# tyb311/TCCT

Measured on AMD Instinct MI355X. Metric: OCT B-scans/sec fwd+bwd(+clip+AdamW), stc_tt bs=8 1x800x1100, higher is better.
Workload: dtype bf16; 1 GPU; stc_tt --los=di bs=8/GPU 1x800x1100 (net tensors 3x800x1104); global_batch=8, parallelism=dp1, ranks=1, grad_allreduce=none, slowest_step=101

## Files before the change

include/tcct_hip.h:

```cpp
#ifndef TCCT_HIP_H
#define TCCT_HIP_H
#include <stdint.h>
#ifdef __cplusplus
extern "C" {
#endif

typedef void* tcct_stream_t;

enum { TCCT_F32 = 0, TCCT_BF16 = 1 };
enum { TCCT_ACT_NONE = 0, TCCT_ACT_LRELU = 1, TCCT_ACT_HSWISH = 2, TCCT_ACT_GELU = 3, TCCT_ACT_SIGMOID = 4,
       TCCT_ACT_ABS = 5 };
enum { TCCT_CRIT_DICE = 0, TCCT_CRIT_DICE2 = 1, TCCT_CRIT_IOU = 2, TCCT_CRIT_MSE = 3 };
enum { TCCT_MCRIT_DICE = 0, TCCT_MCRIT_DICE2 = 1, TCCT_MCRIT_IOU = 2, TCCT_MCRIT_CE = 3 };

int tcct_version(void);
const char* tcct_last_error(void);
int tcct_set_outputs_prezeroed(int on);

int tcct_image_to_nhwc4(const float* img, void* out, int N, int Csrc, int H, int Wsrc, int Wdst, int dtype,
                        tcct_stream_t stream);
int tcct_u8_gather2d(const uint8_t* src, uint8_t* dst, int N, int SH, int SW, int C, int sy0, int sx0, int sh, int sw, int DH, int DW,
                     int dy0, int dx0, int dh, int dw, int flipy, int flipx, int mul, int div, int fill, tcct_stream_t stream);
int tcct_onehot_to_index(const int64_t* onehot, uint8_t* lab, int N, int C, int64_t HW, tcct_stream_t stream);
int tcct_labels_to_u8(const int64_t* lab, uint8_t* out, int N, int H, int Wsrc, int Wdst, tcct_stream_t stream);
int tcct_nhwc_to_nchw_f32(const void* x, float* y, int N, int64_t HW, int C, int dtype, tcct_stream_t stream);

int tcct_act_fwd(const void* x, void* y, int64_t n, int kind, int dtype, tcct_stream_t stream);
int tcct_act_bwd(const void* x, const void* dy, void* dx, int64_t n, int kind, int dtype, tcct_stream_t stream);
int tcct_add(const void* a, const void* b, void* y, int64_t n, int dtype, tcct_stream_t stream);
int tcct_add_act_fwd(const void* a, const void* b, void* y, int64_t n, int kind, int dtype, tcct_stream_t stream);
int tcct_add_act_bwd(const void* a, const void* b, const void* dy, void* dx, int64_t n, int kind, int dtype,
                     tcct_stream_t stream);
int tcct_residual_fwd(const void* x, const void* z, const float* scale, void* y, int B, int64_t per_sample,
                      int dtype, tcct_stream_t stream);
int tcct_scale_rows(const void* x, const float* scale, void* y, int B, int64_t per_sample, int dtype,
                    tcct_stream_t stream);
int tcct_affine2_add(const void* y1, const float* ab1, const void* y2, const float* ab2, void* z, int64_t M, int C, int dtype, tcct_stream_t stream);
int tcct_add3_scale(const void* a, const void* b, const void* c, void* y, int64_t n, float alpha, int dtype,
                    tcct_stream_t stream);
int tcct_scale(const void* x, void* y, int64_t n, float alpha, int dtype, tcct_stream_t stream);
int tcct_concat2(const void* a, const void* b, void* y, int64_t M, int Ca, int Cb, int dtype, tcct_stream_t stream);
int tcct_split2(const void* dy, void* da, void* db, int64_t M, int Ca, int Cb, int dtype, tcct_stream_t stream);
int tcct_axpy_f32(const float* x, float* y, int64_t n, float alpha, tcct_stream_t stream);

int tcct_bn_stats(const void* x, int64_t M, int C, int pre_act, double* sums , int dtype, tcct_stream_t stream);
int tcct_bn_finalize(const double* sums, int64_t M, int C, const float* gamma, const float* beta, float eps,
                     float momentum, float* running_mean, float* running_var, int64_t* num_batches_tracked,
                     float* mean_rstd , float* ab , tcct_stream_t stream);
int tcct_bn_eval_ab(int C, const float* gamma, const float* beta, float eps, const float* running_mean,
                    const float* running_var, float* mean_rstd, float* ab, tcct_stream_t stream);
int tcct_bn_apply(const void* x, void* y, int64_t M, int C, const float* ab, int pre_act, int post_act, int dtype,
                  tcct_stream_t stream);
int tcct_bn_apply_train(const void* x, const void* res, void* y, int64_t M, int C, const double* sums, const float* gamma,
                        const float* beta, float eps, float momentum, float* running_mean, float* running_var,
                        int64_t* num_batches_tracked, float* mean_rstd, float* ab, int pre_act, int post_act, int dtype,
                        tcct_stream_t stream);
int tcct_bn_pool_fwd_train(const void* x, void* z, void* pooled, void* amax, int N, int H, int W, int C, const double* sums, const float* gamma,
                           const float* beta, float eps, float momentum, float* running_mean, float* running_var,
                           int64_t* num_batches_tracked, float* mean_rstd, float* ab, int pre_act, int post_act, int dtype,
                           tcct_stream_t stream);
int tcct_bn_pool_bwd(const void* x, const void* dpool, const void* dskip, const void* amax, void* dx, int N, int H, int W, int C, const float* mean_rstd,
                     const float* ab, int pre_act, int post_act, double* sums, float* dgamma, float* dbeta, int dtype, tcct_stream_t stream);
int tcct_bn_apply_add(const void* x, const void* res, void* y, int64_t M, int C, const float* ab, int pre_act, int post_act, int dtype,
                      tcct_stream_t stream);
int tcct_bn_bwd_reduce(const void* x, const void* dy, int64_t M, int C, const float* mean_rstd, const float* ab,
                       int pre_act, int post_act, double* sums , int dtype, tcct_stream_t stream);
int tcct_bn_bwd_apply(const void* x, const void* dy, void* dx, int64_t M, int C, const float* mean_rstd,
                      const float* ab, const float* gamma, const double* sums, int pre_act, int post_act,
                      float* dgamma, float* dbeta, int dtype, tcct_stream_t stream);
int tcct_bn_bwd_coef(const double* sums, int raw, int64_t M, int C, const float* mean_rstd, const float* ab, float* coef, float* dgamma,
                     float* dbeta, tcct_stream_t stream);
int tcct_bn_bwd_reduce2_raw(const void* y1, const void* y2, const void* dz, int64_t M, int C, double* raw1, double* raw2, int dtype, tcct_stream_t stream);
int tcct_bn_sums_from_raw(const double* raw, const float* mean_rstd, int C, double* sums, tcct_stream_t stream);

int tcct_bn2_add_act_fwd(const void* xa, const void* xb, void* y, int64_t M, int C, const float* abA, const float* abB, int pre_act,
                         int act, int dtype, tcct_stream_t stream);
int tcct_bn2_add_act_train(const void* xa, const void* xb, void* y, int64_t M, int C, const double* sumsA, const float* gammaA,
                           const float* betaA, float* running_meanA, float* running_varA, int64_t* nbtA, float* mean_rstdA,
                           float* abA, const double* sumsB, const float* gammaB, const float* betaB, float* running_meanB,
                           float* running_varB, int64_t* nbtB, float* mean_rstdB, float* abB, float eps, float momentum,
                           int pre_act, int act, int dtype, tcct_stream_t stream);
int tcct_bn2_add_act_bwd_reduce(const void* xa, const void* xb, const void* dy, int64_t M, int C, const float* mean_rstdA,
                                const float* abA, const float* mean_rstdB, const float* abB, int pre_act, int act, double* sums,
                                int dtype, tcct_stream_t stream);
int tcct_bn2_add_act_bwd_apply(const void* xa, const void* xb, const void* dy, void* dxa, void* dxb, int64_t M, int C,
                               const float* mean_rstdA, const float* abA, const float* mean_rstdB, const float* abB,
                               const double* sums, int pre_act, int act, float* dgammaA, float* dbetaA, float* dgammaB,
                               float* dbetaB, int dtype, tcct_stream_t stream);

int tcct_layernorm_fwd(const void* x, void* y, int64_t M, int C, const float* gamma, const float* beta, float eps,
                       float* mean_rstd , int dtype, tcct_stream_t stream);
int tcct_layernorm_bwd(const void* x, const void* dy, void* dx, int64_t M, int C, const float* gamma,
                       const float* mean_rstd, float* dgamma, float* dbeta, int dtype, tcct_stream_t stream);
int tcct_layernorm_bwd_add(const void* x, const void* dy, const void* res, void* dx, int64_t M, int C, const float* gamma,
                           const float* mean_rstd, float* dgamma, float* dbeta, int dtype, tcct_stream_t stream);

int tcct_conv2d_fwd(const void* x, const float* w, const float* bias, void* y, int N, int H, int W, int Cin,
                    int Cin_w, int Cout, int KH, int KW, int stride, int padh, int padw, int in_dtype, int out_dtype,
                    tcct_stream_t stream);
int tcct_conv2d_dgrad(const void* dy, const float* w, void* dx, int N, int H, int W, int Cin, int Cout, int KH,
                      int KW, int padh, int padw, int dy_dtype, int dx_dtype, tcct_stream_t stream);
int tcct_conv2d_wgrad(const void* x, const void* dy, float* dw, float* dbias, int N, int H, int W, int Cin,
                      int Cin_w, int Cout, int KH, int KW, int stride, int padh, int padw, int x_dtype, int dy_dtype,
                      tcct_stream_t stream);

int tcct_conv32f_pack_weights(const float* w, float* wp, int KH, int KW, int transposed, tcct_stream_t stream);
int tcct_conv32f_fwd(const float* x, const float* wp, const float* bias, const float* yadd, float* y, int N, int H, int W, int KH, int KW, int PH,
                     int PW, tcct_stream_t stream);
int tcct_conv32f_wgrad(const float* x, const float* dy, float* dw, float* dbias, int N, int H, int W, int KH, int KW, int PH, int PW,
                       tcct_stream_t stream);
int tcct_conv32f_pack_weights_sub(const float* w, float* wp, int KH, int KW, int transposed, int cin_total, int o_off, int i_off, tcct_stream_t stream);
int tcct_conv32f_fwd_strided(const float* x, const float* wp, const float* bias, float* y, int N, int H, int W, int KH, int KW, int PH, int PW, int xs,
                             int xo, int ys, int yo, int accumulate, tcct_stream_t stream);
int tcct_conv32f_wgrad_strided(const float* x, const float* dy, float* dw, float* dbias, int N, int H, int W, int KH, int KW, int PH, int PW, int xs,
                               int xo, int ds, int dof, int ldi, int o_off, int i_off, tcct_stream_t stream);
// ... 296 lines not shown
```

tcct_amd/csrc/norm.hip:

```cpp
#include "common.h"
#include <cstdlib>

#define NB 256
#define NBR 1024
static inline int bn_vec(int C, int dtype) {
    static int v8 = -1;
    if (v8 < 0) v8 = 0;
    return (v8 && dtype == TCCT_BF16 && C % 8 == 0) ? 8 : ((C % 4 == 0) ? 4 : 1);
}

template <int VEC>
__device__ __forceinline__ void bn_block_reduce2(float* sm, const float* s, const float* q, int t, int C, int CV, int R, double* sums) {
#pragma unroll
    for (int pass = 0; pass < 2; ++pass) {
        if (pass) __syncthreads();
#pragma unroll
        for (int k = 0; k < VEC; ++k) sm[t * VEC + k] = pass ? q[k] : s[k];
        __syncthreads();
        if (t < C) {
            double a = 0.0;
            const int cvv = t / VEC, k = t % VEC;
            for (int rr = 0; rr < R; ++rr) a += (double)sm[(rr * CV + cvv) * VEC + k];
            atomicAdd(&sums[pass * C + t], a);
        }
// ... 448 lines not shown
                        float dz = e[q].v[k] + (((am >> (2 * k)) & 3u) == (unsigned)q ? g.v[k] : 0.f);
                        if (POST != TCCT_ACT_NONE) dz *= actg<POST>(post_act, a_[k] * u + b_[k]);
                        s[k] += dz; q2[k] += dz * (u - mu[k]) * rs[k];
                    }
            }
        }
    }
    bn_block_reduce2<4>(sm, s, q2, t, C, C4, R, sums);
}
template <typename T, int PRE, int POST>
__global__ void k_bn_pool_bwd_apply(const T* __restrict__ x, const T* __restrict__ dpool, const T* __restrict__ dskip,
                                    const unsigned char* __restrict__ amax, T* __restrict__ dx, int N, int H, int W, int C,
                                    const float* __restrict__ mean_rstd, const float* __restrict__ ab, const double* __restrict__ sums,
                                    int pre_act, int post_act, float* __restrict__ dgamma, float* __restrict__ dbeta) {
    const int C4 = C >> 2, Ho = H >> 1, Wo = W >> 1;
    const int i = blockIdx.x * blockDim.x + threadIdx.x;
    if (blockIdx.x == 0 && blockIdx.y == 0 && threadIdx.x < C) { dbeta[threadIdx.x] = (float)sums[threadIdx.x]; dgamma[threadIdx.x] = (float)sums[C + threadIdx.x]; }
    if (i >= Wo * C4) return;
    const int wo = i / C4, c0 = (i - wo * C4) * 4;
    const float invM = 1.f / (float)((int64_t)N * H * W);
    float a_[4], b_[4], mu[4], rs[4], s1[4], s2[4];
#pragma unroll
    for (int k = 0; k < 4; ++k) {
        const int c = c0 + k;
        a_[k] = ab[c]; b_[k] = ab[C + c]; mu[k] = mean_rstd[c]; rs[k] = mean_rstd[C + c];
        s1[k] = (float)sums[c] * invM; s2[k] = (float)sums[C + c] * invM;
    }
    for (int row = blockIdx.y; row < N * Ho; row += gridDim.y) {
        const int n = row / Ho, ho = row - n * Ho;
        const int64_t b00 = (((int64_t)n * H + 2 * ho) * W + 2 * wo) * C + c0;
        const int64_t offs[4] = {b00, b00 + C, b00 + (int64_t)W * C, b00 + (int64_t)W * C + C};
        f4 v[4], e[4];
#pragma unroll
        for (int q = 0; q < 4; ++q) { v[q] = ld4(x + offs[q]); e[q] = dskip ? ld4(dskip + offs[q]) : f4zero(); }
        const int64_t p = (int64_t)row * Wo + wo;
        const f4 g = ld4(dpool + p * C + c0);
        const unsigned am = amax[p * C4 + (c0 >> 2)];
#pragma unroll
        for (int q = 0; q < 4; ++q) {
            f4 o;
#pragma unroll
            for (int k = 0; k < 4; ++k) {
                const float u = actf<PRE>(pre_act, v[q].v[k]);
                float dz = e[q].v[k] + (((am >> (2 * k)) & 3u) == (unsigned)q ? g.v[k] : 0.f);
                if (POST != TCCT_ACT_NONE) dz *= actg<POST>(post_act, a_[k] * u + b_[k]);
                const float xh = (u - mu[k]) * rs[k];
                o.v[k] = a_[k] * (dz - s1[k] - xh * s2[k]);
                if (PRE != TCCT_ACT_NONE) o.v[k] *= actg<PRE>(pre_act, v[q].v[k]);
            }
            st4(dx + offs[q], o);
        }
    }
}
static bool bn_pool_ok(int N, int H, int W, int C) { return C % 4 == 0 && C >= 4 && C <= NB && NB % (C / 4) == 0 && H % 2 == 0 && W % 2 == 0 && H >= 2 && W >= 2 && N >= 1; }
static inline dim3 bn_pool_grid(int per_row, int64_t rows) {
    const int gx = (per_row + NB - 1) / NB;
    int64_t gy = ((1 << 14) + gx - 1) / gx;
    if (gy > rows) gy = rows;
    if (gy > 65535) gy = 65535;
    if (gy < 1) gy = 1;
    return dim3((unsigned)gx, (unsigned)gy);
}
#define BN_POOL_KINDS(CALL) do { if (pre_act == TCCT_ACT_LRELU && post_act == TCCT_ACT_NONE) { constexpr int PRE = TCCT_ACT_LRELU, POST = TCCT_ACT_NONE; CALL; } \
                                 else { constexpr int PRE = -1, POST = -1; CALL; } } while (0)
extern "C" int tcct_bn_pool_fwd_train(const void* x, void* z, void* pooled, void* amax, int N, int H, int W, int C, const double* sums,
                                      const float* gamma, const float* beta, float eps, float momentum, float* running_mean,
                                      float* running_var, int64_t* num_batches_tracked, float* mean_rstd, float* ab, int pre_act, int post_act,
                                      int dtype, tcct_stream_t stream) {
    TCCT_CHECK(bn_pool_ok(N, H, W, C), "bn_pool_fwd_train: needs even H, W and C/4 dividing 256 (got %d,%d,%d)", H, W, C);
    TCCT_CHECK(sums && gamma && beta && mean_rstd && ab && amax, "bn_pool_fwd_train: NULL argument");
    BnTrain tr{sums, gamma, beta, eps, momentum, running_mean, running_var, num_batches_tracked, mean_rstd, ab};
    BN_POOL_KINDS(TCCT_DISPATCH(dtype, hipLaunchKernelGGL((k_bn_pool_fwd<T, PRE, POST>), bn_pool_grid((W / 2) * (C / 4), (int64_t)N * (H / 2)), dim3(NB), 0,
                                                          (hipStream_t)stream, (const T*)x, (T*)z, (T*)pooled, (unsigned char*)amax, N, H, W, C, pre_act, post_act, tr)));
    TCCT_LAUNCH_OK();
}
extern "C" int tcct_bn_pool_bwd(const void* x, const void* dpool, const void* dskip, const void* amax, void* dx, int N, int H, int W, int C,
                                const float* mean_rstd, const float* ab, int pre_act, int post_act, double* sums, float* dgamma, float* dbeta,
                                int dtype, tcct_stream_t stream) {
    TCCT_CHECK(bn_pool_ok(N, H, W, C), "bn_pool_bwd: needs even H, W and C/4 dividing 256 (got %d,%d,%d)", H, W, C);
    TCCT_CHECK(dpool != nullptr && amax != nullptr, "bn_pool_bwd: dpool / amax is NULL");
    hipStream_t st = (hipStream_t)stream;
    if (!tcct_skip_zero_fill() && hipMemsetAsync(sums, 0, sizeof(double) * 2 * C, st) != hipSuccess) { tcct_set_error("bn_pool_bwd: memset failed"); return -2; }
    const int64_t rows = (int64_t)N * (H / 2);
    const int gr = rows < 512 ? (int)rows : 512;
    BN_POOL_KINDS(TCCT_DISPATCH(dtype, hipLaunchKernelGGL((k_bn_pool_bwd_reduce<T, PRE, POST>), dim3(gr), dim3(NBR), 0, st, (const T*)x, (const T*)dpool,
                                                          (const T*)dskip, (const unsigned char*)amax, N, H, W, C, mean_rstd, ab, pre_act, post_act, sums)));
    BN_POOL_KINDS(TCCT_DISPATCH(dtype, hipLaunchKernelGGL((k_bn_pool_bwd_apply<T, PRE, POST>), bn_pool_grid((W / 2) * (C / 4), rows), dim3(NB), 0, st, (const T*)x,
                                                          (const T*)dpool, (const T*)dskip, (const unsigned char*)amax, (T*)dx, N, H, W, C, mean_rstd, ab, sums,
                                                          pre_act, post_act, dgamma, dbeta)));
    TCCT_LAUNCH_OK();
}

#define LN_MAXCH 3
#ifndef LN_TOK
#define LN_TOK 1
#endif
template <typename T, int NCH>
__global__ void k_ln_fwd(const T* __restrict__ x, T* __restrict__ y, int64_t M, int C, const float* __restrict__ gamma,
                         const float* __restrict__ beta, float eps, float* __restrict__ mean_rstd) {
    const int C4 = C >> 2;
    const int lane = threadIdx.x & 15;
    const int64_t grp = ((int64_t)blockIdx.x * blockDim.x + threadIdx.x) >> 4;
    const int64_t ngrp = ((int64_t)gridDim.x * blockDim.x) >> 4;
    float gam[NCH][4], bet[NCH][4];
#pragma unroll
    for (int j = 0; j < NCH; ++j)
#pragma unroll
        for (int k = 0; k < 4; ++k) {
            const int ch = lane + 16 * j;
            gam[j][k] = ch < C4 ? gamma[ch * 4 + k] : 0.f; bet[j][k] = ch < C4 ? beta[ch * 4 + k] : 0.f;
        }
    for (int64_t m0 = grp * LN_TOK; m0 < M; m0 += ngrp * LN_TOK) {
        f4 v[LN_TOK][NCH];
#pragma unroll
        for (int t = 0; t < LN_TOK; ++t)
#pragma unroll
            for (int j = 0; j < NCH; ++j) {
                const int ch = lane + 16 * j;
                if (ch < C4 && m0 + t < M) v[t][j] = ld4(x + (m0 + t) * C + ch * 4); else v[t][j] = f4zero();
            }
#pragma unroll
        for (int t = 0; t < LN_TOK; ++t) {
            const int64_t m = m0 + t;
            float s = 0.f;
#pragma unroll
            for (int j = 0; j < NCH; ++j) s += v[t][j].v[0] + v[t][j].v[1] + v[t][j].v[2] + v[t][j].v[3];
            s = row16_sum(s);
            float mean = s / (float)C, q = 0.f;
#pragma unroll
            for (int j = 0; j < NCH; ++j) {
                int ch = lane + 16 * j;
                if (ch < C4) {
#pragma unroll
                    for (int k = 0; k < 4; ++k) { float d = v[t][j].v[k] - mean; q += d * d; }
                }
            }
            q = row16_sum(q);
            float rstd = rsqrtf(q / (float)C + eps);
            if (m < M) {
                if (lane == 0) { mean_rstd[2 * m] = mean; mean_rstd[2 * m + 1] = rstd; }
#pragma unroll
                for (int j = 0; j < NCH; ++j) {
                    int ch = lane + 16 * j;
                    if (ch < C4) {
// ... 299 lines not shown
```

tcct_amd/ops.py:

```python
import os
import weakref

import torch

from ._lib import lib, dtype_code, TcctError, launch_on, F32, BF16

ACT = {None: 0, 'none': 0, 'lrelu': 1, 'hswish': 2, 'gelu': 3, 'sigmoid': 4, 'abs': 5}


class _ZeroPool:

    def __init__(self):
        self.buf = None
        self.off = 0
        self.active = False
        self.frozen = False

    def begin(self, device, nbytes=8 << 20):
        if self.buf is None or self.buf.device != device or self.buf.numel() < nbytes:
            if self.frozen:
                raise TcctError('the zero pool cannot be re-allocated after a training step was captured into a hipGraph '
                                f'(pool on {self.buf.device}, step on {device})')
            self.buf = torch.empty(nbytes, device=device, dtype=torch.uint8)
        self.buf.zero_()
# ... 107 lines not shown
        lib.bilinear_bwd_x2(int(BILINEAR_BWD_X2))
        _BILINEAR_X2_SET[0] = BILINEAR_BWD_X2
    fpl_lazy_grad_reset()
    _pack_evict()
    _pack_all(device)
    _STEP['main'] = torch.cuda.current_stream(device)
    for v in _STEP['marks'].values():
        v[0] = v[1] = 0


_STEP = {'main': None, 'marks': {}, 'listener': None}


def set_grad_mark_listener(fn):
    _STEP['listener'] = fn
    _STEP['marks'].clear()


def step_streams():
    out = [] if _STEP['main'] is None else [_STEP['main']]
    for v in _SIDE_STREAMS.values():
        out.append(v[0] if isinstance(v, tuple) else v)
    return out


class _FastFunction(torch.autograd.Function):

    @classmethod
    def apply(cls, *args):
        return super(torch.autograd.Function, cls).apply(*args)


class _GradMark(_FastFunction):
    @staticmethod
    def forward(ctx, x, key):
        ctx.key = key
        return x.view_as(x)

    @staticmethod
    def backward(ctx, dy):
        cnt = _STEP['marks'].get(ctx.key)
        fn = _STEP['listener']
        if cnt is not None and fn is not None:
            cnt[1] += 1
            if cnt[1] == cnt[0]:
                fn(ctx.key)
        return dy, None


def grad_mark(x, key):
    if _STEP['listener'] is None or not ZERO.active or not (torch.is_grad_enabled() and x.requires_grad):
        return x
    _STEP['marks'].setdefault(key, [0, 0])[0] += 1
    return _GradMark.apply(x, key)


def end_step():
    ZERO.end()
    if _WGRAD_USED:
        cur = torch.cuda.current_stream()
        for st in _WGRAD_USED.values():
            cur.wait_stream(st)
        _WGRAD_USED.clear()
    _WGRAD_KEEP.clear()


_WGRAD_USED = {}
_WGRAD_KEEP = []
DW_WGRAD_SIDE = True


def fresh_stream(device=None, avoid=()):
    taken = {torch.cuda.current_stream(device).cuda_stream}
    for v in _SIDE_STREAMS.values():
        taken.add((v[0] if isinstance(v, tuple) else v).cuda_stream)
    for st in avoid:
        taken.add(st.cuda_stream)
    for _ in range(64):
        st = torch.cuda.Stream(device=device)
        if st.cuda_stream not in taken:
            return st
    raise TcctError('fresh_stream: no stream of the pool is free of aliases')


class _wgrad_stream:
    def __init__(self, enable, *tensors):
        self.enable, self.tensors = enable, tensors

    def __enter__(self):
        if not self.enable:
            return self
        cur = torch.cuda.current_stream()
        key = ('wgrad', cur.device.index)
        ent = _SIDE_STREAMS.get(key)
        if ent is None:
            ent = _SIDE_STREAMS[key] = (fresh_stream(cur.device), torch.cuda.Event())
        self.side, ev = ent
        ev.record(cur)
        self.side.wait_event(ev)
        self.ctx = launch_on(self.side)
        self.ctx.__enter__()
        return self

    def __exit__(self, *exc):
        if not self.enable:
            return False
        self.ctx.__exit__(*exc)
# ... 1007 lines not shown

    @staticmethod
    def backward(ctx, dl, _dv):
        v, skip, wa, wb = ctx.saved_tensors
        w1, b1, w2, b2, w3, b3 = ctx.params
        N_, H, W_, C, Ho, Wo, align, nc = ctx.cfg
        dl = _as(dl, torch.float32)
        dev = v.device
        M = N_ * Ho * Wo
        dv, dskip = torch.empty_like(v), torch.empty_like(skip)
        F32_, BF_ = dtype_code(torch.float32), dtype_code(v.dtype)
        lib.conv2d_dgrad(dl, wa, dv, N_, Ho, Wo, 32, nc, 1, 1, 0, 0, F32_, BF_)
        lib.conv2d_dgrad(dl, wb, dskip, N_, Ho, Wo, 32, nc, 1, 1, 0, 0, F32_, BF_)
        dy = torch.empty((N_, H, W_, C), device=dev, dtype=v.dtype)
        lib.bilinear_bwd(dv, dy, N_, H, W_, C, Ho, Wo, align, BF_)
        params = (w1, b1, w2, b2, w3, b3)
        with _wgrad_stream(_slot_written(*params), v, skip, dl, wa, wb):
            dwa, dwb = ZERO.get((nc, 32), torch.float32, dev), ZERO.get((nc, 32), torch.float32, dev)
            dccc = ZERO.get((nc,), torch.float32, dev)
            lib.pw_wgrad_smalln(v, dl, dwa, dccc, M, 32, nc, BF_, F32_)
            lib.pw_wgrad_smalln(skip, dl, dwb, None, M, 32, nc, BF_, F32_)
            outs = [_grad_out(p, tuple(p.shape)) for p in params]
            lib.tail_compose3_bwd(w1, b1, w2, b2, w3, nc, dwa, dwb, dccc, *outs)
        return (dy, dskip) + tuple(_ret(o, p) for o, p in zip(outs, params)) + (None,)


class _UpSkipConvT32AuxLow(_FastFunction):

    @staticmethod
    def forward(ctx, y, skip, w1, b1, w2, b2, w3, b3, align):
        _chk(y, skip, w1, b1, w2, b2, w3, b3)
        N_, H, W_, C = y.shape
        _, Ho, Wo, _ = skip.shape
        dev, nc = y.device, w3.shape[0]
        F32_ = dtype_code(torch.float32)
        wcc = torch.empty((nc, 64), device=dev, dtype=torch.float32)
        wa8 = torch.zeros((8, 32, 1, 1), device=dev, dtype=torch.float32)
        wa, wb = wa8[:nc], torch.empty((nc, 32, 1, 1), device=dev, dtype=torch.float32)
        ccc = torch.empty(nc, device=dev, dtype=torch.float32)
        lib.tail_compose3(w1, b1, w2, b2, w3, b3, nc, wcc, wa, wb, ccc)
        lg = torch.empty((N_, Ho, Wo, nc), device=dev, dtype=torch.float32)
        if HEAD_UPADD and align and Ho == 2 * H and Wo == 2 * W_:
            z8 = torch.empty((N_, H, W_, 8), device=dev, dtype=torch.float32)
            lib.pw_fwd(y, wa8, None, z8, N_ * H * W_, 32, 8, 0, F32_)
            lib.pw_fwd_f32_upadd(skip, wb, ccc, lg, N_, H, W_, 32, nc, z8)
        else:
            z = torch.empty((N_, H, W_, nc), device=dev, dtype=torch.float32)
            lib.pw_fwd(y, wa, None, z, N_ * H * W_, 32, nc, 0, F32_)
            lib.pw_fwd(skip, wb, ccc, lg, N_ * Ho * Wo, 32, nc, 0, F32_)
            lib.bilinear_add_fwd(z, lg, lg, N_, H, W_, nc, Ho, Wo, int(align), F32_)
        ctx.save_for_backward(y, skip, wa, wb)
        ctx.params = (w1, b1, w2, b2, w3, b3)
        ctx.cfg = (N_, H, W_, C, Ho, Wo, int(align), nc)
        return lg

    @staticmethod
    def backward(ctx, dl):
        y, skip, wa, wb = ctx.saved_tensors
        N_, H, W_, C, Ho, Wo, align, nc = ctx.cfg
        dl = _as(dl, torch.float32)
        dev = y.device
        F32_, BF_ = dtype_code(torch.float32), dtype_code(y.dtype)
        dz = torch.empty((N_, H, W_, nc), device=dev, dtype=torch.float32)
        lib.bilinear_bwd(dl, dz, N_, H, W_, nc, Ho, Wo, align, F32_)
        dy, dskip = torch.empty_like(y), torch.empty_like(skip)
        lib.conv2d_dgrad(dz, wa, dy, N_, H, W_, 32, nc, 1, 1, 0, 0, F32_, BF_)
        lib.conv2d_dgrad(dl, wb, dskip, N_, Ho, Wo, 32, nc, 1, 1, 0, 0, F32_, BF_)
        params = ctx.params
        with _wgrad_stream(_slot_written(*params), y, skip, dl, dz, wa, wb):
            dwa, dwb = ZERO.get((nc, 32), torch.float32, dev), ZERO.get((nc, 32), torch.float32, dev)
            dccc = ZERO.get((nc,), torch.float32, dev)
            lib.pw_wgrad_smalln(y, dz, dwa, None, N_ * H * W_, 32, nc, BF_, F32_)
            lib.pw_wgrad_smalln(skip, dl, dwb, dccc, N_ * Ho * Wo, 32, nc, BF_, F32_)
            outs = [_grad_out(p, tuple(p.shape)) for p in params]
            lib.tail_compose3_bwd(params[0], params[1], params[2], params[3], params[4], nc, dwa, dwb, dccc, *outs)
        return (dy, dskip) + tuple(_ret(o, p) for o, p in zip(outs, params)) + (None,)


HEAD_UPADD = True
TAIL_AUX_LOW = True


def up_skip_conv_t32_aux_low(y, skip, w1, b1, w2, b2, w3, b3, align_corners=True):
    return _UpSkipConvT32AuxLow.apply(y, skip, w1, b1, w2, b2, w3, b3, bool(align_corners))


def up_skip_conv_t32_from_y(y, skip, w1, b1, w2, b2, align_corners=True):
    with torch.no_grad():
        N_, H, W_, C = y.shape
        v = torch.empty_like(skip)
        lib.bilinear_fwd(y, v, N_, H, W_, C, skip.shape[1], skip.shape[2], int(align_corners), dtype_code(y.dtype))
    return up_skip_conv_t32_from_v(v, skip, w1, b1, w2, b2)


TAIL_AUX = True


def up_skip_conv_t32_aux_ok(y, skip, w1, b1, w2, b2, w3, b3):
    return (TAIL_AUX and up_skip_conv_t32_ok(y, skip, w1, b1, w2, b2) and w3.dim() == 4 and tuple(w3.shape[1:]) == (32, 1, 1) and 2 <= w3.shape[0] <= 8
            and b3 is not None and w3.is_contiguous())


def up_skip_conv_t32_aux(y, skip, w1, b1, w2, b2, w3, b3, align_corners=True):
    return _UpSkipConvT32Aux.apply(y, skip, w1, b1, w2, b2, w3, b3, bool(align_corners))


def up_skip_conv_t32_from_v(v, skip, w1, b1, w2, b2):
    with torch.no_grad():
        wc = torch.empty((32, 64), device=v.device, dtype=torch.float32)
        c = torch.empty(32, device=v.device, dtype=torch.float32)
        lib.tail_compose(w1, b1, w2, b2, wc, c)
        g = torch.empty_like(skip)
        lib.pw_fwd_cat2(v, skip, 32, wc, c, g, v.numel() // 32, 64, 32, None, 0)
    return g


class _HeadThroughT32(_FastFunction):

    @staticmethod
    def forward(ctx, s, wt, bt, wa, ba):
        _chk(s, wt, bt, wa, ba)
        N_, H, W_, _ = s.shape
        dev, nc = s.device, wa.shape[0]
        wh = torch.empty((nc, 32, 1, 1), device=dev, dtype=torch.float32)
        ch = torch.empty(nc, device=dev, dtype=torch.float32)
        lib.head_compose(wt, bt, wa, ba, nc, wh, ch)
        lg = torch.empty((N_, H, W_, nc), device=dev, dtype=torch.float32)
        lib.pw_fwd(s, wh, ch, lg, N_ * H * W_, 32, nc, 0, dtype_code(torch.float32))
        ctx.save_for_backward(s, wh)
        ctx.params = (wt, bt, wa, ba)
        return lg

    @staticmethod
# ... 539 lines not shown
    return (BN_DEFER and BN_FUSE and bn_training and torch.is_grad_enabled() and x.dtype == torch.bfloat16 and x.dim() == 4 and x.shape[-1] in (64, 96)
            and ACT[post_act] == ACT['hswish'] and x.numel() * 2 < 2 ** 31)


def batchnorm_deferred(x, gamma, beta, running_mean, running_var, num_batches_tracked, eps, momentum, post_act):
    link = BnLink(None, None, ACT[post_act])
    y = _BatchNormDeferred.apply(x, gamma, beta, running_mean, running_var, num_batches_tracked, float(eps), float(momentum), ACT[post_act], link)
    return y, link


def pw_conv_bn_ok(x, w, bias, bn_training, pre_act, post_act, x2=None, prev=None):
    if not (BN_FUSE and bn_training and torch.is_grad_enabled() and ACT[pre_act] == 0):
        return False
    if x.dtype != torch.bfloat16 or x.dim() != 4 or not x.is_cuda or (w.dim() == 4 and tuple(w.shape[2:]) != (1, 1)):
        return False
    K = x.shape[-1] + (x2.shape[-1] if x2 is not None else 0)
    N = w.shape[0]
    if x2 is not None and not (x.shape[-1] == 64 and x2.shape == x.shape and x2.dtype == x.dtype):
        return False
    M = x.numel() // x.shape[-1]
    if w.shape[1] != K or M * max(K, N) * 2 >= 2 ** 31:
        return False
    return bool(lib.pw_bwd_bn_supported(K, N, ACT[post_act], -1 if prev is None else prev.post, 1 if x2 is not None else 0))


def pw_conv_bn(x, w, bias, bn, post_act=None, residual=None, fork=False, x2=None, x_final=False, deferred=None, defer_apply=False):
    gamma, beta, rm, rv, nbt, eps, mom = bn
    link = BnLink(None, None, ACT[post_act])
    w4 = w.view(w.shape[0], w.shape[1], 1, 1) if w.dim() == 2 else w
    if deferred is not None:
        if post_act is not None or fork or x2 is not None or x.shape[-1] != w.shape[0] or x.shape[-1] not in (64, 96):
            raise TcctError('pw_conv_bn(deferred=...): square 64 / 96 convolution without activation, fork or concatenation only')
        prev = deferred if (x.shape[-1] == 64 and BN_FUSE_RED) else None
        out = _PwConvBN.apply(x, None, w4, bias, gamma, beta, rm, rv, nbt, float(eps), float(mom), 0, residual, False, link, prev, deferred.ab)
        out._bn_link = link
        return out
    prev = _bn_link_of(x, x_final)
    if prev is not None and not pw_conv_bn_ok(x, w, bias, True, None, post_act, x2, prev):
        prev = None
    if defer_apply:
        if residual is not None or x2 is not None or ACT[post_act] not in (ACT['hswish'], ACT['none']):
            raise TcctError('pw_conv_bn(defer_apply=True): BatchNorm (+ Hardswish) without residual / concatenation only')
        out = _PwConvBN.apply(x, None, w4, bias, gamma, beta, rm, rv, nbt, float(eps), float(mom), ACT[post_act], None, fork, link, prev, None, True)
        return out, link
    out = _PwConvBN.apply(x, x2, w4, bias, gamma, beta, rm, rv, nbt, float(eps), float(mom), ACT[post_act], residual, fork, link, prev)
    z = out[0] if fork else out
    z._bn_link = link
    return out


BN_POOL_FUSE = True


class _BnPoolFork(_FastFunction):

    @staticmethod
    def forward(ctx, x, gamma, beta, rm, rv, nbt, eps, momentum, pre, post):
        ctx.set_materialize_grads(False)
        _chk(x, gamma, beta)
        N, H, W, C = x.shape
        dc = dtype_code(x.dtype)
        fused = getattr(x, '_bn_sums', None)
        if fused is not None and fused[1] == pre and fused[0].numel() == 2 * C:
            sums = fused[0]
        else:
            sums = ZERO.get((2 * C,), torch.float64, x.device)
            lib.bn_stats(x, N * H * W, C, pre, sums, dc)
        mean_rstd = torch.empty(2 * C, device=x.device, dtype=torch.float32)
        ab = torch.empty(2 * C, device=x.device, dtype=torch.float32)
        z = torch.empty_like(x)
        pooled = torch.empty((N, H // 2, W // 2, C), device=x.device, dtype=x.dtype)
        amax = torch.empty((N, H // 2, W // 2, C // 4), device=x.device, dtype=torch.uint8)
        lib.bn_pool_fwd_train(x, z, pooled, amax, N, H, W, C, sums, gamma, beta, eps, momentum, rm, rv, nbt, mean_rstd, ab, pre, post, dc)
        ctx.save_for_backward(x, mean_rstd, ab, amax)
        ctx.cfg = (pre, post, gamma, beta)
        return pooled, z

    @staticmethod
    def backward(ctx, dpool, dskip):
        x, mean_rstd, ab, amax = ctx.saved_tensors
        pre, post, gamma, beta = ctx.cfg
        N, H, W, C = x.shape
        dc = dtype_code(x.dtype)
        if dpool is None and dskip is None:
            return (None,) * 10
        if dpool is None:
            dpool = torch.zeros((N, H // 2, W // 2, C), device=x.device, dtype=x.dtype)
        dpool = _as(dpool, x.dtype)
        if dskip is not None:
            dskip = _as(dskip, x.dtype)
        sums = ZERO.get((2 * C,), torch.float64, x.device)
        dx = torch.empty_like(x)
        dg = _grad_out(gamma) if ZERO.active and getattr(gamma, '_grad_slot', None) is not None else torch.empty(C, device=x.device, dtype=torch.float32)
        db = _grad_out(beta) if ZERO.active and getattr(beta, '_grad_slot', None) is not None else torch.empty(C, device=x.device, dtype=torch.float32)
        lib.bn_pool_bwd(x, dpool, dskip, amax, dx, N, H, W, C, mean_rstd, ab, pre, post, sums, dg, db, dc)
        return dx, _ret(dg, gamma), _ret(db, beta), None, None, None, None, None, None, None


def bn_pool_ok(x, training):
    N, H, W, C = x.shape
    return (BN_POOL_FUSE and training and torch.is_grad_enabled() and x.requires_grad and C % 4 == 0 and C <= 256 and 256 % (C // 4) == 0
            and H % 2 == 0 and W % 2 == 0 and H >= 2 and W >= 2)


def batchnorm_maxpool2_fork(x, gamma, beta, running_mean, running_var, num_batches_tracked=None, eps=1e-5, momentum=0.1, pre_act=None,
                            post_act=None):
    return _BnPoolFork.apply(x, gamma, beta, running_mean, running_var, num_batches_tracked, float(eps), float(momentum), ACT[pre_act], ACT[post_act])


def batchnorm(x, gamma, beta, running_mean, running_var, num_batches_tracked=None, eps=1e-5, momentum=0.1,
              pre_act=None, post_act=None, training=True, residual=None):
    if not training and torch.is_grad_enabled() and x.requires_grad:
        raise TcctError('eval-mode batchnorm is inference-only here')
    link = None
    if (BN_FUSE and training and torch.is_grad_enabled() and x.dtype == torch.bfloat16 and ACT[pre_act] == 0
            and ACT[post_act] in (0, 2) and x.shape[-1] in (64, 96, 128)):
        link = BnLink(None, None, ACT[post_act])
    z = _BatchNorm.apply(x, gamma, beta, running_mean, running_var, num_batches_tracked, float(eps), float(momentum),
                         ACT[pre_act], ACT[post_act], bool(training), residual, link)
    if link is not None:
        z._bn_link = link
    return z


class _Bn2AddAct(_FastFunction):

    @staticmethod
    def forward(ctx, xa, gA, bA, xb, gB, bB, bufs, eps, momentum, pre, act_kind):
        _chk(xa, xb, gA, bA, gB, bB)
        C = xa.shape[-1]
        M = xa.numel() // C
        dc = dtype_code(xa.dtype)
        st, ss = [], []
        for x, g, b, (rm, rv, nbt) in ((xa, gA, bA, bufs[0]), (xb, gB, bB, bufs[1])):
            fused = getattr(x, '_bn_sums', None)
            if fused is not None and fused[1] == pre and fused[0].numel() == 2 * C:
                sums = fused[0]
            else:
                sums = ZERO.get((2 * C,), torch.float64, x.device)
                lib.bn_stats(x, M, C, pre, sums, dc)
            mr = torch.empty(2 * C, device=x.device, dtype=torch.float32)
            ab = torch.empty(2 * C, device=x.device, dtype=torch.float32)
            st += [mr, ab]
            ss.append(sums)
        y = torch.empty_like(xa)
        (rmA, rvA, nbtA), (rmB, rvB, nbtB) = bufs
        lib.bn2_add_act_train(xa, xb, y, M, C, ss[0], gA, bA, rmA, rvA, nbtA, st[0], st[1], ss[1], gB, bB, rmB, rvB, nbtB, st[2], st[3],
                              eps, momentum, pre, act_kind, dc)
        ctx.save_for_backward(xa, xb, *st)
        ctx.cfg = (pre, act_kind)
        ctx.params = (gA, bA, gB, bB)
        return y

    @staticmethod
    def backward(ctx, dy):
        xa, xb, mrA, abA, mrB, abB = ctx.saved_tensors
        pre, act_kind = ctx.cfg
        gA, bA, gB, bB = ctx.params
        dy = _as(dy, xa.dtype)
        C = xa.shape[-1]
# ... 1192 lines not shown
```

Baseline: 423.5 B-scans/s.

## Fuse low-rank skip dgrad into batchnorm-maxpool backward kernels

Instead of materializing the full-resolution skip gradient through a separate 1x1 conv dgrad (nc->32 channels) and reading it back in the BN+pool backward, the head's backward passes a recipe (dl, wb, nc) through a link object attached to the skip tensor. New HIP reduce and apply kernels recompute dskip on the fly from the small nc-channel gradient staged in LDS, rounding to bf16 to match the old path. This removes a full-size bf16 tensor write and read plus a kernel launch. In exchange it adds cross-autograd plumbing through a zero-stride marker tensor and recomputes the tiny matmul in both the reduce and apply passes.

Measured after the change: 429.6 B-scans/s (median of 6 runs). 1.01x the previous value.

```diff
diff --git a/include/tcct_hip.h b/include/tcct_hip.h
--- a/include/tcct_hip.h
+++ b/include/tcct_hip.h
@@ -61,6 +61,9 @@
                            tcct_stream_t stream);
 int tcct_bn_pool_bwd(const void* x, const void* dpool, const void* dskip, const void* amax, void* dx, int N, int H, int W, int C, const float* mean_rstd,
                      const float* ab, int pre_act, int post_act, double* sums, float* dgamma, float* dbeta, int dtype, tcct_stream_t stream);
+int tcct_bn_pool_bwd_lowrank(const void* x, const void* dpool, const float* dl, const float* wb, int nc, const void* amax, void* dx, int N, int H, int W,
+                             int C, const float* mean_rstd, const float* ab, int pre_act, int post_act, double* sums, float* dgamma, float* dbeta,
+                             int dtype, tcct_stream_t stream);
 int tcct_bn_apply_add(const void* x, const void* res, void* y, int64_t M, int C, const float* ab, int pre_act, int post_act, int dtype,
                       tcct_stream_t stream);
 int tcct_bn_bwd_reduce(const void* x, const void* dy, int64_t M, int C, const float* mean_rstd, const float* ab,
diff --git a/tcct_amd/csrc/norm.hip b/tcct_amd/csrc/norm.hip
--- a/tcct_amd/csrc/norm.hip
+++ b/tcct_amd/csrc/norm.hip
@@ -524,6 +524,141 @@
         }
     }
 }
+#define LR_SLOT 256
+template <int NC>
+__device__ __forceinline__ void lowrank_stage(float* __restrict__ slot, const float* __restrict__ dl0 , int64_t row_stride ,
+                                              int nwin , int lane) {
+    wave_lds_fence();
+    if (lane < nwin * NC) {
+        const float2 r0 = reinterpret_cast<const float2*>(dl0)[lane], r1 = reinterpret_cast<const float2*>(dl0 + row_stride)[lane];
+        reinterpret_cast<float2*>(slot)[lane] = r0;
+        reinterpret_cast<float2*>(slot + LR_SLOT / 2)[lane] = r1;
+    }
+    wave_lds_fence();
+}
+template <int NC>
+__device__ __forceinline__ void lowrank_dskip(const float* __restrict__ slot, int wl, const float (&w)[NC][4], f4 (&e)[4]) {
+#pragma unroll
+    for (int rr = 0; rr < 2; ++rr) {
+        float f[2 * NC];
+#pragma unroll
+        for (int i = 0; i < NC; ++i) {
+            const float2 t = reinterpret_cast<const float2*>(slot + rr * (LR_SLOT / 2) + wl * 2 * NC)[i];
+            f[2 * i] = t.x; f[2 * i + 1] = t.y;
+        }
+#pragma unroll
+        for (int col = 0; col < 2; ++col) {
+            float a[4] = {0.f, 0.f, 0.f, 0.f};
+#pragma unroll
+            for (int j = 0; j < NC; ++j)
+#pragma unroll
+                for (int k = 0; k < 4; ++k) a[k] += f[col * NC + j] * w[j][k];
+            const uint32_t lo = pack_bf16x2(a[0], a[1]), hi = pack_bf16x2(a[2], a[3]);
+            f4& o = e[rr * 2 + col];
+            o.v[0] = __uint_as_float(lo << 16); o.v[1] = __uint_as_float(lo & 0xffff0000u);
+            o.v[2] = __uint_as_float(hi << 16); o.v[3] = __uint_as_float(hi & 0xffff0000u);
+        }
+    }
+}
+template <int NC>
+__global__ void __launch_bounds__(NBR) k_bn_pool_bwd_reduce_lr(const bf16* __restrict__ x, const bf16* __restrict__ dpool, const float* __restrict__ dl,
+                                                               const float* __restrict__ wb, const unsigned char* __restrict__ amax, int N, int H, int W,
+                                                               const float* __restrict__ mean_rstd, double* __restrict__ sums) {
+    constexpr int C = 32, C4 = 8, R = NBR / C4;
+    __shared__ __attribute__((aligned(16))) float sm[NBR * 4];
+    const int Ho = H >> 1, Wo = W >> 1;
+    const int t = threadIdx.x, lane = t & 63, wl = lane >> 3, cv = t & 7, c0 = cv * 4;
+    float* slot = sm + (t >> 6) * LR_SLOT;
+    float s[4], q2[4], mu[4], rs[4], w[NC][4];
+#pragma unroll
+    for (int k = 0; k < 4; ++k) { s[k] = q2[k] = 0.f; mu[k] = mean_rstd[c0 + k]; rs[k] = mean_rstd[C + c0 + k]; }
+#pragma unroll
+    for (int j = 0; j < NC; ++j)
+#pragma unroll
+        for (int k = 0; k < 4; ++k) w[j][k] = wb[j * C + c0 + k];
+    for (int row = blockIdx.x; row < N * Ho; row += gridDim.x) {
+        const int n = row / Ho, ho = row - n * Ho;
+        for (int wo0 = (t >> 6) * 8; wo0 < Wo; wo0 += R) {
+            const int wo = wo0 + wl;
+            const int64_t pix0 = ((int64_t)n * H + 2 * ho) * W + 2 * wo0;
+            lowrank_stage<NC>(slot, dl + pix0 * NC, (int64_t)W * NC, min(8, Wo - wo0), lane);
+            if (wo >= Wo) continue;
+            const int64_t b00 = (pix0 + 2 * wl) * C + c0;
+            const int64_t offs[4] = {b00, b00 + C, b00 + (int64_t)W * C, b00 + (int64_t)W * C + C};
+            f4 v[4], e[4];
+#pragma unroll
+            for (int q = 0; q < 4; ++q) v[q] = ld4(x + offs[q]);
+            const int64_t p = (int64_t)row * Wo + wo;
+            const f4 g = ld4(dpool + p * C + c0);
+            const unsigned am = amax[p * C4 + cv];
+            lowrank_dskip<NC>(slot, wl, w, e);
+#pragma unroll
+            for (int q = 0; q < 4; ++q)
+#pragma unroll
+                for (int k = 0; k < 4; ++k) {
+                    const float u = actf<TCCT_ACT_LRELU>(TCCT_ACT_LRELU, v[q].v[k]);
+                    const float dz = e[q].v[k] + (((am >> (2 * k)) & 3u) == (unsigned)q ? g.v[k] : 0.f);
+                    s[k] += dz; q2[k] += dz * (u - mu[k]) * rs[k];
+                }
+        }
+    }
+    __syncthreads();
+    bn_block_reduce2<4>(sm, s, q2, t, C, C4, R, sums);
+}
+template <int NC>
+__global__ void __launch_bounds__(NB) k_bn_pool_bwd_apply_lr(const bf16* __restrict__ x, const bf16* __restrict__ dpool, const float* __restrict__ dl,
+                                                             const float* __restrict__ wb, const unsigned char* __restrict__ amax, bf16* __restrict__ dx,
+                                                             int N, int H, int W, const float* __restrict__ mean_rstd, const float* __restrict__ ab,
+                                                             const double* __restrict__ sums, float* __restrict__ dgamma, float* __restrict__ dbeta) {
+    constexpr int C = 32, C4 = 8;
+    __shared__ __attribute__((aligned(16))) float sm[(NB / 64) * LR_SLOT];
+    const int Ho = H >> 1, Wo = W >> 1;
+    const int i = blockIdx.x * blockDim.x + threadIdx.x, lane = threadIdx.x & 63, wl = lane >> 3;
+    if (blockIdx.x == 0 && blockIdx.y == 0 && threadIdx.x < C) { dbeta[threadIdx.x] = (float)sums[threadIdx.x]; dgamma[threadIdx.x] = (float)sums[C + threadIdx.x]; }
+    const int wo0 = (i - lane) >> 3, wo = wo0 + wl, c0 = (i & 7) * 4;
+    if (wo0 >= Wo) return;
+    float* slot = sm + (threadIdx.x >> 6) * LR_SLOT;
+    const float invM = 1.f / (float)((int64_t)N * H * W);
+    float a_[4], mu[4], rs[4], s1[4], s2[4], w[NC][4];
+#pragma unroll
+    for (int k = 0; k < 4; ++k) {
+        const int c = c0 + k;
+        a_[k] = ab[c]; mu[k] = mean_rstd[c]; rs[k] = mean_rstd[C + c];
+        s1[k] = (float)sums[c] * invM; s2[k] = (float)sums[C + c] * invM;
+    }
+#pragma unroll
+    for (int j = 0; j < NC; ++j)
+#pragma unroll
+        for (int k = 0; k < 4; ++k) w[j][k] = wb[j * C + c0 + k];
+    for (int row = blockIdx.y; row < N * Ho; row += gridDim.y) {
+        const int n = row / Ho, ho = row - n * Ho;
+        const int64_t pix0 = ((int64_t)n * H + 2 * ho) * W + 2 * wo0;
+        lowrank_stage<NC>(slot, dl + pix0 * NC, (int64_t)W * NC, min(8, Wo - wo0), lane);
+        if (wo >= Wo) continue;
+        const int64_t b00 = (pix0 + 2 * wl) * C + c0;
+        const int64_t offs[4] = {b00, b00 + C, b00 + (int64_t)W * C, b00 + (int64_t)W * C + C};
+        f4 v[4], e[4];
+#pragma unroll
+        for (int q = 0; q < 4; ++q) v[q] = ld4(x + offs[q]);
+        const int64_t p = (int64_t)row * Wo + wo;
+        const f4 g = ld4(dpool + p * C + c0);
+        const unsigned am = amax[p * C4 + (c0 >> 2)];
+        lowrank_dskip<NC>(slot, wl, w, e);
+#pragma unroll
+        for (int q = 0; q < 4; ++q) {
+            f4 o;
+#pragma unroll
+            for (int k = 0; k < 4; ++k) {
+                const float u = actf<TCCT_ACT_LRELU>(TCCT_ACT_LRELU, v[q].v[k]);
+                const float dz = e[q].v[k] + (((am >> (2 * k)) & 3u) == (unsigned)q ? g.v[k] : 0.f);
+                const float xh = (u - mu[k]) * rs[k];
+                o.v[k] = a_[k] * (dz - s1[k] - xh * s2[k]);
+                o.v[k] *= actg<TCCT_ACT_LRELU>(TCCT_ACT_LRELU, v[q].v[k]);
+            }
+            st4(dx + offs[q], o);
+        }
+    }
+}
 static bool bn_pool_ok(int N, int H, int W, int C) { return C % 4 == 0 && C >= 4 && C <= NB && NB % (C / 4) == 0 && H % 2 == 0 && W % 2 == 0 && H >= 2 && W >= 2 && N >= 1; }
 static inline dim3 bn_pool_grid(int per_row, int64_t rows) {
     const int gx = (per_row + NB - 1) / NB;
@@ -562,6 +697,31 @@
                                                           pre_act, post_act, dgamma, dbeta)));
     TCCT_LAUNCH_OK();
 }
+static bool bn_pool_bwd_lowrank_ok(int C, int nc, int pre_act, int post_act, int dtype) {
+    return C == 32 && nc >= 2 && nc <= 8 && pre_act == TCCT_ACT_LRELU && post_act == TCCT_ACT_NONE && dtype == TCCT_BF16;
+}
+extern "C" int tcct_bn_pool_bwd_lowrank(const void* x, const void* dpool, const float* dl, const float* wb, int nc, const void* amax, void* dx, int N,
+                                        int H, int W, int C, const float* mean_rstd, const float* ab, int pre_act, int post_act, double* sums,
+                                        float* dgamma, float* dbeta, int dtype, tcct_stream_t stream) {
+    TCCT_CHECK(bn_pool_ok(N, H, W, C), "bn_pool_bwd_lowrank: needs even H, W (got %d,%d,%d)", H, W, C);
+    TCCT_CHECK(bn_pool_bwd_lowrank_ok(C, nc, pre_act, post_act, dtype), "bn_pool_bwd_lowrank: bf16, C=32, nc 2..8, lrelu/none only (C=%d nc=%d)", C, nc);
+    TCCT_CHECK(dpool != nullptr && amax != nullptr && dl != nullptr && wb != nullptr, "bn_pool_bwd_lowrank: NULL argument");
+    TCCT_CHECK(((uintptr_t)dl & 7) == 0, "bn_pool_bwd_lowrank: dl must be 8-byte aligned");
+    hipStream_t st = (hipStream_t)stream;
+    if (!tcct_skip_zero_fill() && hipMemsetAsync(sums, 0, sizeof(double) * 2 * C, st) != hipSuccess) { tcct_set_error("bn_pool_bwd_lowrank: memset failed"); return -2; }
+    const int64_t rows = (int64_t)N * (H / 2);
+    const int gr = rows < 512 ? (int)rows : 512;
+    const dim3 ga = bn_pool_grid((W / 2) * (C / 4), rows);
+#define LR_LAUNCH(NC) case NC: \
+        hipLaunchKernelGGL((k_bn_pool_bwd_reduce_lr<NC>), dim3(gr), dim3(NBR), 0, st, (const bf16*)x, (const bf16*)dpool, dl, wb, (const unsigned char*)amax, N, H, W, \
+                           mean_rstd, sums); \
+        hipLaunchKernelGGL((k_bn_pool_bwd_apply_lr<NC>), ga, dim3(NB), 0, st, (const bf16*)x, (const bf16*)dpool, dl, wb, (const unsigned char*)amax, (bf16*)dx, N, H, W, \
+                           mean_rstd, ab, sums, dgamma, dbeta); \
+        break
+    switch (nc) { LR_LAUNCH(2); LR_LAUNCH(3); LR_LAUNCH(4); LR_LAUNCH(5); LR_LAUNCH(6); LR_LAUNCH(7); LR_LAUNCH(8); }
+#undef LR_LAUNCH
+    TCCT_LAUNCH_OK();
+}
 
 #define LN_MAXCH 3
 #ifndef LN_TOK
diff --git a/tcct_amd/ops.py b/tcct_amd/ops.py
--- a/tcct_amd/ops.py
+++ b/tcct_amd/ops.py
@@ -183,7 +183,11 @@
     if _STEP['listener'] is None or not ZERO.active or not (torch.is_grad_enabled() and x.requires_grad):
         return x
     _STEP['marks'].setdefault(key, [0, 0])[0] += 1
-    return _GradMark.apply(x, key)
+    y = _GradMark.apply(x, key)
+    link = getattr(x, '_skip0', None)
+    if link is not None:
+        y._skip0 = link
+    return y
 
 
 def end_step():
@@ -1297,6 +1301,10 @@
         ctx.save_for_backward(y, skip, wa, wb)
         ctx.params = (w1, b1, w2, b2, w3, b3)
         ctx.cfg = (N_, H, W_, C, Ho, Wo, int(align), nc)
+        link = getattr(skip, '_skip0', None) if SKIP0_LOWRANK else None
+        ctx.skip0 = link if (link is not None and link.ok and 2 <= nc <= 8 and ctx.needs_input_grad[1] and not grad_is_watched(skip)) else None
+        if ctx.skip0 is not None:
+            del link.recipes[:]
         return lg
 
     @staticmethod
@@ -1308,9 +1316,15 @@
         F32_, BF_ = dtype_code(torch.float32), dtype_code(y.dtype)
         dz = torch.empty((N_, H, W_, nc), device=dev, dtype=torch.float32)
         lib.bilinear_bwd(dl, dz, N_, H, W_, nc, Ho, Wo, align, F32_)
-        dy, dskip = torch.empty_like(y), torch.empty_like(skip)
+        dy = torch.empty_like(y)
         lib.conv2d_dgrad(dz, wa, dy, N_, H, W_, 32, nc, 1, 1, 0, 0, F32_, BF_)
-        lib.conv2d_dgrad(dl, wb, dskip, N_, Ho, Wo, 32, nc, 1, 1, 0, 0, F32_, BF_)
+        if ctx.skip0 is not None:
+            marker = torch.zeros(1, device=dev, dtype=skip.dtype)
+            ctx.skip0.recipes.append((marker, dl, wb, nc))
+            dskip = marker.expand(skip.shape)
+        else:
+            dskip = torch.empty_like(skip)
+            lib.conv2d_dgrad(dl, wb, dskip, N_, Ho, Wo, 32, nc, 1, 1, 0, 0, F32_, BF_)
         params = ctx.params
         with _wgrad_stream(_slot_written(*params), y, skip, dl, dz, wa, wb):
             dwa, dwb = ZERO.get((nc, 32), torch.float32, dev), ZERO.get((nc, 32), torch.float32, dev)
@@ -1324,6 +1338,7 @@
 
 HEAD_UPADD = True
 TAIL_AUX_LOW = True
+SKIP0_LOWRANK = True
 
 
 def up_skip_conv_t32_aux_low(y, skip, w1, b1, w2, b2, w3, b3, align_corners=True):
@@ -1969,14 +1984,26 @@
 BN_POOL_FUSE = True
 
 
+class Skip0Link:
+    __slots__ = ('ok', 'recipes')
+
+    def __init__(self, ok):
+        self.ok, self.recipes = bool(ok), []
+
+
+def bn_pool_lowrank_ok(x, pre, post):
+    return x.dtype == torch.bfloat16 and x.shape[-1] == 32 and pre == ACT['lrelu'] and post == ACT['none']
+
+
 class _BnPoolFork(_FastFunction):
 
     @staticmethod
-    def forward(ctx, x, gamma, beta, rm, rv, nbt, eps, momentum, pre, post):
+    def forward(ctx, x, gamma, beta, rm, rv, nbt, eps, momentum, pre, post, link=None):
         ctx.set_materialize_grads(False)
         _chk(x, gamma, beta)
         N, H, W, C = x.shape
         dc = dtype_code(x.dtype)
+        ctx.link = link
         fused = getattr(x, '_bn_sums', None)
         if fused is not None and fused[1] == pre and fused[0].numel() == 2 * C:
             sums = fused[0]
@@ -2000,7 +2027,19 @@
         N, H, W, C = x.shape
         dc = dtype_code(x.dtype)
         if dpool is None and dskip is None:
-            return (None,) * 10
+            return (None,) * 11
+        recipes = []
+        if ctx.link is not None:
+            recipes, ctx.link.recipes = ctx.link.recipes, []
+        lowrank = None
+        if len(recipes) == 1 and dskip is not None and dskip.dim() == 4 and dskip.stride(0) == 0 and dskip.data_ptr() == recipes[0][0].data_ptr():
+            lowrank, dskip = recipes[0], None
+        elif recipes:
+            dskip = None if dskip is None else _as(dskip, x.dtype)
+            for _, dl, wb, nc in recipes:
+                d = torch.empty_like(x)
+                lib.conv2d_dgrad(dl, wb, d, N, H, W, C, nc, 1, 1, 0, 0, dtype_code(torch.float32), dc)
+                dskip = d if dskip is None else add(dskip, d)
         if dpool is None:
             dpool = torch.zeros((N, H // 2, W // 2, C), device=x.device, dtype=x.dtype)
         dpool = _as(dpool, x.dtype)
@@ -2010,8 +2049,13 @@
         dx = torch.empty_like(x)
         dg = _grad_out(gamma) if ZERO.active and getattr(gamma, '_grad_slot', None) is not None else torch.empty(C, device=x.device, dtype=torch.float32)
         db = _grad_out(beta) if ZERO.active and getattr(beta, '_grad_slot', None) is not None else torch.empty(C, device=x.device, dtype=torch.float32)
-        lib.bn_pool_bwd(x, dpool, dskip, amax, dx, N, H, W, C, mean_rstd, ab, pre, post, sums, dg, db, dc)
-        return dx, _ret(dg, gamma), _ret(db, beta), None, None, None, None, None, None, None
+        if lowrank is not None:
+            _, dl, wb, nc = lowrank
+            keep_until_end_of_step(dl, wb, torch.cuda.current_stream())
+            lib.bn_pool_bwd_lowrank(x, dpool, dl, wb, nc, amax, dx, N, H, W, C, mean_rstd, ab, pre, post, sums, dg, db, dc)
+        else:
+            lib.bn_pool_bwd(x, dpool, dskip, amax, dx, N, H, W, C, mean_rstd, ab, pre, post, sums, dg, db, dc)
+        return dx, _ret(dg, gamma), _ret(db, beta), None, None, None, None, None, None, None, None
 
 
 def bn_pool_ok(x, training):
@@ -2022,7 +2066,10 @@
 
 def batchnorm_maxpool2_fork(x, gamma, beta, running_mean, running_var, num_batches_tracked=None, eps=1e-5, momentum=0.1, pre_act=None,
                             post_act=None):
-    return _BnPoolFork.apply(x, gamma, beta, running_mean, running_var, num_batches_tracked, float(eps), float(momentum), ACT[pre_act], ACT[post_act])
+    link = Skip0Link(bn_pool_lowrank_ok(x, ACT[pre_act], ACT[post_act]))
+    pooled, z = _BnPoolFork.apply(x, gamma, beta, running_mean, running_var, num_batches_tracked, float(eps), float(momentum), ACT[pre_act], ACT[post_act], link)
+    z._skip0 = link
+    return pooled, z
 
 
 def batchnorm(x, gamma, beta, running_mean, running_var, num_batches_tracked=None, eps=1e-5, momentum=0.1,
```
